# MircoWerner/VkRadixSort

Measured on AMD Instinct MI355X. Metric: Gkeys/s sorting 10^8 uint32 at 1/2/4/8 MI355X; % of HBM roofline, higher is better.
Workload: dtype u32

## Files before the change

vkradixsort_amd/csrc/vrs_contract.hip:

```cpp
#include "vrs_device.hpp"
#include "vrs_key_order.hpp"

#include <algorithm>
#include <cstdio>
#include <cstdlib>
#include <type_traits>

namespace vrs {

__device__ __forceinline__ void histogram_count(uint32_t *s_hist, uint32_t key, uint32_t shift, bool valid) {
    const uint32_t d = digit_of(key, shift);
    const uint64_t active = __ballot(valid);
    if (active == 0) return;
    const uint32_t first = static_cast<uint32_t>(__ffsll(static_cast<long long>(active))) - 1u;
    const uint32_t d0 = __builtin_amdgcn_readlane(d, first);
    const uint64_t same = __ballot(valid && d == d0);
    if (same == active) {
        if (lane_id() == first) atomicAdd(&s_hist[d0], static_cast<uint32_t>(__popcll(active)));
    } else if (valid) {
        atomicAdd(&s_hist[d], 1u);
    }
}

template <typename K, typename DG>
// ... 261 lines not shown
#pragma unroll
        for (int u = 0; u < kDepth; ++u) {
            if (r + u < q1) o[static_cast<size_t>(r + u) * kBins] = run;
            run += t[u];
        }
    }
}

constexpr uint32_t kFusedMaxChunks = 48;

template <typename K, int ITEMS, int WAVES, bool PAIRS, int RANK, int OCC, bool SPLIT = false>
__global__ __launch_bounds__(WAVES * 64, OCC) void scatter_kernel(const K *__restrict__ keys_in,
                                                             K *__restrict__ keys_out,
                                                             const uint32_t *__restrict__ values_in,
                                                             uint32_t *__restrict__ values_out,
                                                             const uint32_t *__restrict__ offsets, uint32_t n,
                                                             uint32_t shift, uint32_t W, uint32_t B, int xcd_remap,
                                                             const uint32_t *__restrict__ tile_order,
                                                             uint32_t offset_row_stride,
                                                             const K *__restrict__ splitters, uint32_t num_splitters) {
    using DG = typename std::conditional<SPLIT, SplitDigit<K>, RadixDigit<K>>::type;
    __shared__ ChunkSmem<K, ITEMS, WAVES, PAIRS> sm;
    __shared__ K s_split[SPLIT ? 256 : 1];
    DG dg;
    if constexpr (SPLIT) {
        stage_splitters(s_split, splitters, num_splitters);
        dg.splitters = s_split;
        dg.count = num_splitters;
    } else {
        dg.shift = shift;
    }
    const uint32_t w = tile_order ? tile_order[blockIdx.x]
                                  : (xcd_remap ? xcd_contiguous_tile(blockIdx.x, W) : blockIdx.x);
    const uint64_t tile_begin = static_cast<uint64_t>(w) * B * kThreads;
    if (tile_begin >= n) return;
    const uint64_t tile_keys = static_cast<uint64_t>(B) * kThreads;
    const uint32_t tile_len = static_cast<uint32_t>(tile_begin + tile_keys <= n ? tile_keys : n - tile_begin);
    uint32_t run_off =
        threadIdx.x < kBins ? offsets[static_cast<size_t>(w) * offset_row_stride * kBins + threadIdx.x] : 0u;
    constexpr uint32_t kChunk = ITEMS * WAVES * 64;
    const bool stream_in = static_cast<size_t>(n) * sizeof(K) >= kStreamInBytes;
    for (uint32_t c0 = 0; c0 < tile_len; c0 += kChunk) {
        const uint32_t valid = min(kChunk, tile_len - c0);
        const K *kin = keys_in + tile_begin + c0;
        const uint32_t *vin = PAIRS ? values_in + tile_begin + c0 : nullptr;
        if (valid == kChunk)
// ... 315 lines not shown
```

vkradixsort_amd/csrc/vrs_device.hpp:

```cpp
#pragma once
#include "vrs_kernels.h"

#include <hip/hip_ext.h>

#include <type_traits>

#define VRS_LAUNCH(kernel, grid, block, stream, ev, ...)                                                        \
    do {                                                                                                        \
        if ((ev).start != nullptr || (ev).stop != nullptr)                                                      \
            hipExtLaunchKernelGGL(kernel, grid, block, 0, stream, (ev).start, (ev).stop, 0, __VA_ARGS__);       \
        else                                                                                                    \
            hipLaunchKernelGGL(kernel, grid, block, 0, stream, __VA_ARGS__);                                    \
    } while (0)

#ifndef VRS_MARK
#define VRS_MARK(i)
#define VRS_MARK_FLUSH()
#endif
namespace vrs {

constexpr size_t kStreamInBytes = size_t(128) << 20;

constexpr int kDtUnroll = 8;
constexpr int kLbItems = 16;
constexpr int kLbBatch = 4;
constexpr int kLbWaves = 8;

constexpr int kBins = 256;
constexpr int kThreads = 256;
constexpr int kWaves = kThreads / 64;

__device__ __forceinline__ uint32_t lane_id() {
    return __builtin_amdgcn_mbcnt_hi(~0u, __builtin_amdgcn_mbcnt_lo(~0u, 0u));
}

__device__ __forceinline__ uint32_t opaque(uint32_t x) {
    asm volatile("" : "+v"(x));
    return x;
}

// ... 248 lines not shown
    mutable bool reserved_yet = false;

    __device__ __forceinline__ void publish(uint32_t v) const {
        if (reserved_yet) return;
        reserved_yet = true;
        const uint32_t cnt = v - pad_keys;
        if (cnt) {
            if (foreign) {
                const uint32_t taken = cnt + __hip_atomic_fetch_add(back, cnt, __ATOMIC_RELAXED, __HIP_MEMORY_SCOPE_AGENT);
                reserved = region_len >= taken ? region_len - taken : 0u;
            } else
                reserved = __hip_atomic_fetch_add(cursor, cnt, __ATOMIC_RELAXED, __HIP_MEMORY_SCOPE_WORKGROUP);
        }
    }
    __device__ __forceinline__ void fetch(int, uint32_t (&)[kLbBatch]) const {}
    __device__ __forceinline__ uint32_t resolve(uint32_t (&)[kLbBatch], bool &) const { return reserved; }
};

template <typename K, typename DG>
__device__ __forceinline__ void recount_keys(uint32_t *cnt, const K *keys, uint32_t count, const DG &dg) {
    for (uint32_t j = threadIdx.x; j < count; j += blockDim.x) atomicAdd(&cnt[dg(keys[j])], 1u);
}

template <typename K, int ITEMS, int WAVES, bool PAIRS, int RANK, bool FULL, typename DG, typename LB = NoLookback, typename SRC = NoPieces>
__device__ __forceinline__ void scatter_chunk(ChunkSmem<K, ITEMS, WAVES, PAIRS> &sm, const K *kin,
                                              const uint32_t *vin, K *kout, uint32_t *vout,
                                              uint32_t valid, const DG &dg, uint32_t &run_off, const LB lb = {},
                                              const SRC src = {}, bool stream_in = false) {
    constexpr uint32_t THREADS = WAVES * 64;
    const uint32_t tid = threadIdx.x;
    const uint32_t lane = tid & 63u;
    const uint32_t wave = tid >> 6;

    VRS_MARK(0);
    K key[ITEMS];
    uint32_t val[PAIRS ? ITEMS : 1];
    const uint32_t seg = wave * (ITEMS * 64) + lane;
    if (FULL && !SRC::kEnabled && stream_in) {
#pragma unroll
        for (int i = 0; i < ITEMS; ++i) key[i] = __builtin_nontemporal_load(kin + seg + i * 64);
        if constexpr (PAIRS) {
#pragma unroll
            for (int i = 0; i < ITEMS; ++i) val[i] = __builtin_nontemporal_load(vin + seg + i * 64);
        }
    } else if constexpr (SRC::kEnabled) {
        uint32_t vs[ITEMS];
#pragma unroll
        for (int i = 0; i < ITEMS; ++i) vs[i] = src.first_slot;
#pragma unroll 1
        for (uint32_t p = src.p0; p < src.p1; ++p) {
            const uint32_t lo = __builtin_amdgcn_readlane(src.lo, p), len = __builtin_amdgcn_readlane(src.len, p), vd = __builtin_amdgcn_readlane(src.slot, p);
#pragma unroll
            for (int i = 0; i < ITEMS; ++i) {
                const uint32_t idx = seg + i * 64;
                vs[i] = idx - lo < len ? vd + (idx - lo) : vs[i];
            }
        }
#pragma unroll
        for (int i = 0; i < ITEMS; ++i) {
            const K k = *src.at(vs[i]);
            key[i] = (FULL || seg + i * 64 < valid) ? k : dg.template pad<K>();
        }
        if constexpr (PAIRS) {
#pragma unroll
            for (int i = 0; i < ITEMS; ++i) val[i] = *src.val_at(vs[i]);
        }
    } else {
#pragma unroll
        for (int i = 0; i < ITEMS; ++i) {
            const uint32_t idx = seg + i * 64;
            if constexpr (FULL) {
                key[i] = kin[idx];
            } else {
                const K k = kin[idx < valid ? idx : valid - 1u];
                key[i] = idx < valid ? k : dg.template pad<K>();
            }
        }
        if constexpr (PAIRS) {
#pragma unroll
            for (int i = 0; i < ITEMS; ++i) {
                const uint32_t idx = seg + i * 64;
                val[i] = vin[FULL ? idx : (idx < valid ? idx : valid - 1u)];
            }
        }
    }
    {
        uint32_t *z = &sm.whist[0][0];
#pragma unroll
        for (int v = 0; v < 4; ++v) z[v * THREADS + tid] = 0;
        if constexpr (LB::kEnabled) {
            if (tid == 0) sm.lb_gave_up = 0;
        }
    }
    __syncthreads();
    VRS_MARK(1);

    uint32_t rank[ITEMS];
    uint32_t *my_hist = sm.whist[wave];
    if constexpr (RANK == RANK_ATOMIC) {
#pragma unroll
        for (int i = 0; i < ITEMS; ++i) {
            const uint32_t d = dg(key[i]);
            const uint32_t d0 = __builtin_amdgcn_readfirstlane(d);
            if (__ballot(d == d0) == ~0ull) {
                uint32_t old = 0;
                if (lane == 0u)
                    old = __hip_atomic_fetch_add(&my_hist[d0], 64u, __ATOMIC_RELAXED, __HIP_MEMORY_SCOPE_WORKGROUP);
                rank[i] = __builtin_amdgcn_readfirstlane(old) + lane;
// ... 111 lines not shown
        lb.template store<K, ITEMS, THREADS, FULL>(sm.gbase, key, dst, kout, valid, dg);
    } else {
#pragma unroll
        for (int i = 0; i < ITEMS; ++i) {
            if (FULL || i * THREADS + tid < valid) kout[dst[i]] = key[i];
        }
    }
    VRS_MARK(5);

    if constexpr (PAIRS) {
#pragma unroll
        for (int i = 0; i < ITEMS; ++i) val[i] = sm.vals[i * THREADS + tid];
        if constexpr (LB::kPool) {
            lb.template store_values<ITEMS, THREADS, FULL>(val, dst, vout, valid);
        } else {
#pragma unroll
            for (int i = 0; i < ITEMS; ++i) {
                if (FULL || i * THREADS + tid < valid) vout[dst[i]] = val[i];
            }
        }
    }
}

constexpr uint32_t kMsdBits = 14, kMsdBuckets = 1u << kMsdBits;
constexpr uint32_t kMsdMinShift = 13, kMsdMaxShift = 18;
constexpr uint32_t kMsdProbeWord = kMsdBuckets + 8u * 256u, kMsdOverWord = kMsdProbeWord + 1u;
constexpr uint32_t kMsdSubBits = kMsdBits - 8, kMsdSub = 1u << kMsdSubBits;

struct BitsDigit {
    uint32_t shift, mask, base;
    __device__ __forceinline__ uint32_t operator()(uint32_t key) const { return ((key - base) >> shift) & mask; }
    __device__ __forceinline__ uint32_t operator()(uint64_t key) const { return static_cast<uint32_t>(key >> shift) & mask; }
    template <typename KK>
    __device__ __forceinline__ KK pad() const { return sizeof(KK) == 4 ? static_cast<KK>(base - 1u) : static_cast<KK>(~static_cast<KK>(0)); }
};

}
```

vkradixsort_amd/csrc/vrs_msd_pool.hip:

```cpp
#include "vrs_local_sort.hpp"

#include <algorithm>
#include <cmath>

namespace vrs {

namespace {

constexpr uint32_t kPoolMinShift = 13, kPoolMaxShift = 18;
constexpr float kPoolSigmas = 6.0f;

__global__ __launch_bounds__(256) void pool_sample_kernel(const uint32_t *__restrict__ keys, uint32_t n, uint32_t key_base,
                                                          PoolStreams ps, PoolPlan *__restrict__ pool, uint32_t top_bits) {
    constexpr int kPerWave = kPoolSampleTiles / 4;
    constexpr int kLoads = kPoolSampleKeys / 64;
    __shared__ uint32_t s_hist[2][256];
    __shared__ uint32_t s_or;
    const uint32_t tid = threadIdx.x, lane = tid & 63u, wave = tid >> 6;
    s_hist[0][tid] = 0;
    s_hist[1][tid] = 0;
    if (tid == 0) s_or = 0;
    const uint32_t t0 = blockIdx.x * kPoolSampleTiles;
    const uint32_t s0 = t0 / ps.tiles_per_stream;
    uint32_t k[kPerWave][kLoads];
// ... 106 lines not shown
    static constexpr bool kPool = true;
    bool foreign = false;
    uint32_t recounted = 0;
    int index = 0;
    const void *stream_keys = nullptr;
    uint32_t done = 0;
    uint32_t seed = 0;
    uint32_t *cursor = nullptr;
    const uint32_t *region = nullptr;
    uint32_t pad_keys = 0;
    uint32_t n_virt = 0;
    uint32_t *overflow = nullptr;
    uint32_t overflow_last = 0;
    uint32_t *gbase2 = nullptr, *split = nullptr, *flags = nullptr;
    uint32_t *fail_word = nullptr;
    mutable uint32_t reserved = 0, cnt = 0, rb = 0, rc = 0, ob = 0, oc = 0;
    mutable bool reserved_yet = false;

    __device__ __forceinline__ void publish(uint32_t v) const {
        if (reserved_yet) return;
        reserved_yet = true;
        cnt = v - pad_keys;
        if (cnt) reserved = __hip_atomic_fetch_add(cursor, cnt, __ATOMIC_RELAXED, __HIP_MEMORY_SCOPE_WORKGROUP);
        rb = region[0];
        rc = region[8 * 256];
        ob = region[16 * 256];
        oc = region[24 * 256];
    }
    __device__ __forceinline__ void fetch(int, uint32_t (&)[kLbBatch]) const {}
    __device__ __forceinline__ uint32_t resolve(uint32_t (&)[kLbBatch], bool &) const { return reserved; }
    __device__ __forceinline__ void refuse() const {}
    __device__ __forceinline__ void place(uint32_t *gbase, uint32_t tid, uint32_t, uint32_t excl) const { place_run(gbase, tid, reserved, excl); }
    __device__ __forceinline__ void place_run(uint32_t *gbase, uint32_t tid, uint32_t reserved, uint32_t excl) const {
        const uint32_t end = reserved + cnt;
        uint32_t g, g2 = 0, sp = 0xFFFFFFFFu;
        bool bad = false;
        if (end <= rc) {
            g = rb + reserved - excl;
        } else if (reserved >= rc) {
            bad = end - rc > oc;
            g = n_virt + ob + (reserved - rc) - excl;
        } else {
            bad = end - rc > oc;
            sp = excl + (rc - reserved);
            g = rb + reserved - excl;
            g2 = n_virt + ob - sp;
            atomicOr(flags, 1u);
        }
        if (cnt && bad) __hip_atomic_fetch_or(fail_word, 1u, __ATOMIC_RELAXED, __HIP_MEMORY_SCOPE_AGENT);
        gbase[tid] = g;
        gbase2[tid] = g2;
        split[tid] = sp;
    }
    template <typename K, int ITEMS, uint32_t THREADS, bool FULL, typename DG>
    __device__ __forceinline__ void store(const uint32_t *, const K (&key)[ITEMS], uint32_t (&dst)[ITEMS], K *kout, uint32_t valid, const DG &dg) const {
        const uint32_t tid = threadIdx.x;
        if (*flags & 1u) {
#pragma unroll
            for (int i = 0; i < ITEMS; ++i) {
                const uint32_t d = dg(key[i]);
                if (i * THREADS + tid >= split[d]) dst[i] = gbase2[d] + (i * THREADS + tid);
            }
        }
#pragma unroll
        for (int i = 0; i < ITEMS; ++i) {
            K *p = dst[i] < n_virt ? kout + dst[i] : overflow + min(dst[i] - n_virt, overflow_last);
            if (FULL || i * THREADS + tid < valid) *p = key[i];
        }
    }
    uint32_t *overflow_values = nullptr;
    template <int ITEMS, uint32_t THREADS, bool FULL>
    __device__ __forceinline__ void store_values(const uint32_t (&val)[ITEMS], const uint32_t (&dst)[ITEMS], uint32_t *vout, uint32_t valid) const {
        const uint32_t tid = threadIdx.x;
#pragma unroll
        for (int i = 0; i < ITEMS; ++i) {
            uint32_t *p = dst[i] < n_virt ? vout + dst[i] : overflow_values + min(dst[i] - n_virt, overflow_last);
            if (FULL || i * THREADS + tid < valid) *p = val[i];
        }
    }
};

struct PoolLookback : StreamLookback {
    static constexpr bool kPool = true;
    PoolReserve at;
    __device__ __forceinline__ void publish(uint32_t v) const {
        if (!at.reserved_yet) {
            at.reserved_yet = true;
            at.cnt = v - at.pad_keys;
            if (at.cnt) __hip_atomic_fetch_add(at.cursor, at.cnt, __ATOMIC_RELAXED, __HIP_MEMORY_SCOPE_WORKGROUP);
            at.rb = at.region[0];
            at.rc = at.region[8 * 256];
            at.ob = at.region[16 * 256];
            at.oc = at.region[24 * 256];
        }
        StreamLookback::publish(v);
    }
    __device__ __forceinline__ void refuse() const { __hip_atomic_fetch_or(at.fail_word, 1u, __ATOMIC_RELAXED, __HIP_MEMORY_SCOPE_AGENT); }
    __device__ __forceinline__ void place(uint32_t *gbase, uint32_t tid, uint32_t before, uint32_t excl) const { at.place_run(gbase, tid, before, excl); }
    template <typename K, int ITEMS, uint32_t THREADS, bool FULL, typename DG>
    __device__ __forceinline__ void store(const uint32_t *g, const K (&key)[ITEMS], uint32_t (&dst)[ITEMS], K *kout, uint32_t valid, const DG &dg) const {
        at.template store<K, ITEMS, THREADS, FULL>(g, key, dst, kout, valid, dg);
    }
    template <int ITEMS, uint32_t THREADS, bool FULL>
    __device__ __forceinline__ void store_values(const uint32_t (&val)[ITEMS], const uint32_t (&dst)[ITEMS], uint32_t *vout, uint32_t valid) const {
        at.template store_values<ITEMS, THREADS, FULL>(val, dst, vout, valid);
    }
};

__device__ __forceinline__ uint32_t xcc_place(unsigned long long xcc_map) {
    const uint32_t my_xcc = xcc_id();
    uint32_t x = 8u;
#pragma unroll
    for (uint32_t q = 0; q < 8u; ++q)
        if (x == 8u && xcc_of(xcc_map, q) == my_xcc) x = q;
    return x;
}

template <bool PAIRS>
__global__ __launch_bounds__(512, 4) void pool_pass_a_kernel(const uint32_t *__restrict__ keys_in, uint32_t *__restrict__ keys_out,
                                                             uint32_t *__restrict__ overflow, uint32_t n, uint32_t key_base,
                                                             PoolStreams ps, PoolPlan *__restrict__ pool, MsdPlan *__restrict__ msd,
                                                             unsigned long long xcc_map, int misplace, uint32_t overflow_capacity, uint32_t par,
                                                             PoolPayloads pv, uint32_t top_bits) {
    __shared__ ChunkSmem<uint32_t, 16, 8, PAIRS> sm;
    __shared__ uint32_t s_gbase2[kBins], s_split[kBins], s_flags;
    if (pool->armed == 0u) return;
    const uint32_t i = blockIdx.x >> 3;
    const uint32_t s_out = xcc_place(xcc_map);
    if (s_out == 8u) {
        if (threadIdx.x == 0) __hip_atomic_fetch_or(&pool->fail[par], 1u, __ATOMIC_RELAXED, __HIP_MEMORY_SCOPE_AGENT);
        return;
    }
    if (threadIdx.x == 0) __hip_atomic_fetch_add(&pool->claim_a[s_out * kPoolMaxTilesA + i], 1u, __ATOMIC_RELAXED, __HIP_MEMORY_SCOPE_WORKGROUP);
    const uint32_t s_in = (s_out + (misplace ? (i & 1u) : 0u)) & 7u;
    const uint32_t len = ps.len[s_in];
    const uint32_t done = i * kPoolTile;
    if (done >= len) return;
    if (threadIdx.x == 0) s_flags = 0;
    const uint32_t valid = min(kPoolTile, len - done);
    const uint32_t *kin = keys_in + ps.start[s_in] + done;
    const uint32_t d = threadIdx.x & 255u;
    RadixDigit<uint32_t> dg;
    dg.shift = pool->shift + (kMsdBits - top_bits);
    dg.base = key_base;
    PoolReserve at;
    at.cursor = &msd->cursor_a[s_out][d];
    at.region = &pool->base[s_out][d];
    at.pad_keys = d == dg(dg.template pad<uint32_t>()) ? kPoolTile - valid : 0u;
    at.n_virt = n;
    at.overflow = overflow;
    at.overflow_last = overflow_capacity - 1u;
    at.gbase2 = s_gbase2;
    at.split = s_split;
    at.flags = &s_flags;
    at.fail_word = &pool->fail[par];
    uint32_t unused = 0;
    const bool stream_in = static_cast<size_t>(n) * sizeof(uint32_t) >= kStreamInBytes;
    if constexpr (PAIRS) {
        at.overflow_values = pv.overflow_values;
        PoolLookback lb;
        lb.at = at;
        lb.stream_keys = keys_in + ps.start[s_in];
        lb.done = done;
        lb.col = pv.status + static_cast<size_t>(s_out) * kBins + d;
        lb.stride = static_cast<size_t>(8) * kBins;
        lb.index = static_cast<int>(i);
        lb.tag = 1u << kLbTagShift;
        lb.budget = pv.spin_budget;
        lb.hold = pv.hold_tile >= 0 && i == static_cast<uint32_t>(pv.hold_tile);
        const uint32_t *vin = pv.values_home + ps.start[s_in] + done;
        if (valid == kPoolTile)
            scatter_chunk<uint32_t, 16, 8, true, RANK_ATOMIC, true>(sm, kin, vin, keys_out, pv.values_partner, valid, dg, unused, lb, NoPieces{}, stream_in);
        else
            scatter_chunk<uint32_t, 16, 8, true, RANK_ATOMIC, false>(sm, kin, vin, keys_out, pv.values_partner, valid, dg, unused, lb);
    } else {
        if (valid == kPoolTile)
            scatter_chunk<uint32_t, 16, 8, false, RANK_ATOMIC, true>(sm, kin, nullptr, keys_out, nullptr, valid, dg, unused, at, NoPieces{}, stream_in);
        else
            scatter_chunk<uint32_t, 16, 8, false, RANK_ATOMIC, false>(sm, kin, nullptr, keys_out, nullptr, valid, dg, unused, at);
    }
}

constexpr float kPoolR = 40.0f;
template <uint32_t SUB>
__device__ __forceinline__ uint32_t pool_space(uint32_t c) {
    if (c == 0u) return 0u;
    const float x = static_cast<float>(c), s = static_cast<float>(SUB);
    return (c + static_cast<uint32_t>(kPoolSigmas * sqrtf(s * kPoolR * (x + s * kPoolR))) + SUB * (kPoolRoomFloor + 4u) + 3u) & ~3u;
}
template <uint32_t SUBBITS, bool GROUPED>
__global__ __launch_bounds__(512) void pool_plan_kernel(MsdPlan *__restrict__ msd, PoolPlan *__restrict__ pool, uint32_t n, uint32_t tiles_b_cap,
                                                       uint32_t slack_capacity, const uint32_t *__restrict__ regions, const uint32_t *__restrict__ overflow,
                                                       uint32_t key_base, PoolStreams ps, PoolGroups groups, uint32_t par, uint32_t keep, uint32_t top_bits) {
    constexpr uint32_t THREADS = 512, WAVES = THREADS / 64, SUB = 1u << SUBBITS, PER = SUB / 64u;
    __shared__ uint32_t s_c[kBins];
    __shared__ uint32_t s_red[4][WAVES];
    __shared__ uint32_t s_hist[WAVES][SUB];
    __shared__ uint2 s_piece[16];
    __shared__ uint32_t s_first[17];
    __shared__ uint32_t s_bad;
    const uint32_t tid = threadIdx.x, lane = tid & 63u, wave = tid >> 6, a = blockIdx.x;
    const uint32_t shift = GROUPED ? 18u : pool->shift, bshift = shift + kMsdBits - top_bits - SUBBITS;
    if (!GROUPED && tid < 256u) {
// ... 194 lines not shown
                                 ? 1u
                                 : 0u;
            pool->max_bucket = 0;
            pool->fail[par ^ 1u] = 0;
            if constexpr (GROUPED) pool->shift = shift;
            msd->shift = shift;
            msd->sub_bits = SUBBITS;
            msd->ok = 0;
        }
    }
}

struct SlackReserve {
    static constexpr bool kEnabled = true;
    static constexpr bool kReserves = true;
    static constexpr bool kPool = true;
    bool foreign = false;
    uint32_t recounted = 0;
    int index = 0;
    const void *stream_keys = nullptr;
    uint32_t done = 0;
    uint32_t seed = 0;
    uint32_t *cursor = nullptr;
    uint32_t start = 0, cap = 0;
    uint32_t local_cap = 0;
    uint32_t *max_bucket = nullptr;
    uint32_t dump = 0;
    uint32_t pad_keys = 0;
    uint32_t above = 0, key_base = 0;
    uint32_t *fail_word = nullptr;
    mutable uint32_t reserved = 0, cnt = 0;
    mutable bool reserved_yet = false;

    __device__ __forceinline__ void publish(uint32_t v) const {
        if (reserved_yet) return;
        reserved_yet = true;
        cnt = v - pad_keys;
        if (cnt) reserved = __hip_atomic_fetch_add(cursor, cnt, __ATOMIC_RELAXED, __HIP_MEMORY_SCOPE_WORKGROUP);
    }
    __device__ __forceinline__ void fetch(int, uint32_t (&)[kLbBatch]) const {}
    __device__ __forceinline__ uint32_t resolve(uint32_t (&)[kLbBatch], bool &) const { return reserved; }
    __device__ __forceinline__ void refuse() const {}
    __device__ __forceinline__ void place(uint32_t *gbase, uint32_t tid, uint32_t, uint32_t excl) const { place_run(gbase, tid, reserved, excl); }
    __device__ __forceinline__ void place_run(uint32_t *gbase, uint32_t tid, uint32_t reserved, uint32_t excl) const {
        const uint32_t end = reserved + cnt;
        const bool bad = cnt != 0u && end > cap;
        if (bad) {
            __hip_atomic_fetch_or(fail_word, 1u, __ATOMIC_RELAXED, __HIP_MEMORY_SCOPE_AGENT);
        } else if (cnt != 0u && end > local_cap) {
            __hip_atomic_fetch_or(fail_word, 2u, __ATOMIC_RELAXED, __HIP_MEMORY_SCOPE_AGENT);
            __hip_atomic_fetch_max(max_bucket, end, __ATOMIC_RELAXED, __HIP_MEMORY_SCOPE_AGENT);
        }
        gbase[tid] = (bad ? dump : start + reserved) - excl;
    }
    template <typename K, int ITEMS, uint32_t THREADS, bool FULL, typename DG>
    __device__ __forceinline__ void store(const uint32_t *, const K (&key)[ITEMS], uint32_t (&dst)[ITEMS], K *kout, uint32_t valid, const DG &) const {
        const uint32_t tid = threadIdx.x;
        uint32_t over = 0;
#pragma unroll
        for (int i = 0; i < ITEMS; ++i) {
            if (FULL || i * THREADS + tid < valid) {
                over |= (key[i] - key_base) & above;
                kout[dst[i]] = key[i];
            }
        }
        if (__ballot(over != 0u) != 0ull && (tid & 63u) == 0u) __hip_atomic_fetch_or(fail_word, 1u, __ATOMIC_RELAXED, __HIP_MEMORY_SCOPE_AGENT);
    }
    template <int ITEMS, uint32_t THREADS, bool FULL>
    __device__ __forceinline__ void store_values(const uint32_t (&val)[ITEMS], const uint32_t (&dst)[ITEMS], uint32_t *vout, uint32_t valid) const {
// ... 14 lines not shown
            if (at.cnt) __hip_atomic_fetch_add(at.cursor, at.cnt, __ATOMIC_RELAXED, __HIP_MEMORY_SCOPE_WORKGROUP);
        }
        StreamLookback::publish(v);
    }
    __device__ __forceinline__ void refuse() const { __hip_atomic_fetch_or(at.fail_word, 1u, __ATOMIC_RELAXED, __HIP_MEMORY_SCOPE_AGENT); }
    __device__ __forceinline__ void place(uint32_t *gbase, uint32_t tid, uint32_t before, uint32_t excl) const { at.place_run(gbase, tid, before, excl); }
    template <typename K, int ITEMS, uint32_t THREADS, bool FULL, typename DG>
    __device__ __forceinline__ void store(const uint32_t *g, const K (&key)[ITEMS], uint32_t (&dst)[ITEMS], K *kout, uint32_t valid, const DG &dg) const {
        at.template store<K, ITEMS, THREADS, FULL>(g, key, dst, kout, valid, dg);
    }
    template <int ITEMS, uint32_t THREADS, bool FULL>
    __device__ __forceinline__ void store_values(const uint32_t (&val)[ITEMS], const uint32_t (&dst)[ITEMS], uint32_t *vout, uint32_t valid) const {
        at.template store_values<ITEMS, THREADS, FULL>(val, dst, vout, valid);
    }
};

template <uint32_t SUBBITS, bool PAIRS>
__global__ __launch_bounds__(512, PAIRS ? 4 : 6) void pool_pass_b_kernel(const uint32_t *__restrict__ regions, const uint32_t *__restrict__ overflow,
                                                             uint32_t *__restrict__ slack, const MsdPlan *__restrict__ msd, PoolPlan *__restrict__ pool,
                                                             uint32_t n_virt, uint32_t key_base, uint32_t local_cap, uint32_t dump,
                                                             unsigned long long xcc_map, uint32_t stamp, uint32_t grouped, uint32_t par, PoolPayloads pv,
                                                             uint32_t top_bits) {
    __shared__ ChunkSmem<uint32_t, 16, 8, PAIRS> sm;
    const uint32_t x = xcc_place(xcc_map), j = blockIdx.x >> 3;
    if (pool->ok_a == 0u) return;
    if (x == 8u) {
        if (threadIdx.x == 0) __hip_atomic_fetch_or(&pool->fail[par], 1u, __ATOMIC_RELAXED, __HIP_MEMORY_SCOPE_AGENT);
        return;
    }
    uint32_t claimed = 0;
    if (threadIdx.x == 0) claimed = __hip_atomic_exchange(&pool->claim_b[j * 8u + x], stamp, __ATOMIC_RELAXED, __HIP_MEMORY_SCOPE_WORKGROUP);
    const uint2 entry = pool->tile_map[x][j < kPoolMaxTilesB ? j : 0u];
    if (j >= pool->tiles_b[x][32]) return;
    const uint32_t a = entry.y & 255u, tile_lo = (entry.y >> 8) * kPoolTile;
    const bool one_piece = entry.x != kPoolTileGeneral;
    const uint32_t lane = threadIdx.x & 63u;
    uint2 pc = make_uint2(0, 0);
    if (!one_piece) pc = pool->pieces[a][lane & 15u];
    const uint32_t shift = pool->shift;
    constexpr uint32_t SUB = 1u << SUBBITS;
    const uint32_t d = threadIdx.x & 255u, b = a * SUB + min(d, SUB - 1u);
    SlackReserve at;
    at.cursor = &pool->sub_cursor[b];
    if (threadIdx.x < SUB) {
        at.start = pool->sub_start[b];
        at.cap = pool->sub_start[b + 1u] - at.start;
    }
    at.local_cap = local_cap;
    at.max_bucket = &pool->max_bucket;
    const uint32_t pend = pc.x, pslot = pc.y;
    const uint32_t before = __shfl_up(pend, 1);
    const uint32_t plo = lane == 0u ? 0u : before;
    const uint32_t plen = lane < 16u ? pend - plo : 0u;
    const uint32_t keys_a = __builtin_amdgcn_readlane(pend, 15);
    const uint32_t valid = one_piece ? kPoolTile : min(kPoolTile, keys_a - tile_lo);
    const unsigned long long touch = __ballot(plen != 0u && plo < tile_lo + valid && pend > tile_lo);
    PieceSrc src;
    src.p0 = static_cast<uint32_t>(__builtin_ctzll(touch | (1ull << 63)));
    src.p1 = 64u - static_cast<uint32_t>(__builtin_clzll(touch | 1ull));
    src.lo = plo - tile_lo;
    src.len = plen;
    src.slot = pslot;
    src.regions = regions;
    src.overflow = overflow;
    src.n_virt = n_virt;
    const uint32_t slot0 = one_piece ? entry.x : __builtin_amdgcn_readlane(pslot, src.p0) + (tile_lo - __builtin_amdgcn_readlane(plo, src.p0));
    src.first_slot = slot0;
    const BitsDigit dg{shift + kMsdBits - top_bits - SUBBITS, SUB - 1u, key_base};
    at.dump = dump;
    at.pad_keys = d == SUB - 1u ? kPoolTile - valid : 0u;
    at.above = grouped ? 0xFF000000u : (shift + kMsdBits < 32u ? ~0u << (shift + kMsdBits) : 0u);
    at.key_base = grouped ? key_base + (a << 24) : key_base;
    at.fail_word = &pool->fail[par];
    uint32_t unused = 0;
    if (threadIdx.x == 0 && claimed == stamp) __hip_atomic_fetch_or(&pool->fail[par], 1u, __ATOMIC_RELAXED, __HIP_MEMORY_SCOPE_AGENT);
    const bool stream_in = static_cast<size_t>(pool->top_base[256]) * sizeof(uint32_t) >= kStreamInBytes;
    const uint32_t *kin = slot0 < n_virt ? regions + slot0 : overflow + (slot0 - n_virt);
    if constexpr (PAIRS) {
        src.vregions = pv.values_partner;
        src.voverflow = pv.overflow_values;
        SlackLookback lb;
        lb.at = at;
        lb.col = pv.status + (static_cast<size_t>(j - (entry.y >> 8)) * 8u + x) * kBins + d;
        lb.stride = static_cast<size_t>(8) * kBins;
        lb.index = static_cast<int>(entry.y >> 8);
        lb.tag = 6u << kLbTagShift;
        lb.budget = pv.spin_budget;
        const uint32_t *vin = slot0 < n_virt ? pv.values_partner + slot0 : pv.overflow_values + (slot0 - n_virt);
        if (one_piece)
            scatter_chunk<uint32_t, 16, 8, true, RANK_ATOMIC, true, BitsDigit, SlackLookback>(sm, kin, vin, slack, pv.slack_values, valid, dg, unused, lb, NoPieces{}, stream_in);
        else if (valid == kPoolTile)
            scatter_chunk<uint32_t, 16, 8, true, RANK_ATOMIC, true, BitsDigit, SlackLookback, PieceSrc>(sm, nullptr, nullptr, slack, pv.slack_values, valid, dg, unused, lb, src);
        else
            scatter_chunk<uint32_t, 16, 8, true, RANK_ATOMIC, false, BitsDigit, SlackLookback, PieceSrc>(sm, nullptr, nullptr, slack, pv.slack_values, valid, dg, unused, lb, src);
    } else {
        if (one_piece)
            scatter_chunk<uint32_t, 16, 8, false, RANK_ATOMIC, true, BitsDigit, SlackReserve>(sm, kin, nullptr, slack, nullptr, valid, dg, unused, at, NoPieces{}, stream_in);
        else if (valid == kPoolTile)
            scatter_chunk<uint32_t, 16, 8, false, RANK_ATOMIC, true, BitsDigit, SlackReserve, PieceSrc>(sm, nullptr, nullptr, slack, nullptr, valid, dg, unused, at, src);
        else
            scatter_chunk<uint32_t, 16, 8, false, RANK_ATOMIC, false, BitsDigit, SlackReserve, PieceSrc>(sm, nullptr, nullptr, slack, nullptr, valid, dg, unused, at, src);
    }
}

}


hipError_t launch_pool_sample(hipStream_t stream, const PoolSampleArgs &a, LaunchEvents ev) {
    const uint32_t *keys = a.keys;
    const uint32_t n = a.form.n, key_base = a.form.key_base, overflow_capacity = a.overflow_capacity, par = a.form.par, top_bits = a.form.top_bits;
    const PoolStreams &ps = a.form.ps;
    PoolPlan *pool = a.form.pool;
    if (n == 0 || ps.tiles_per_stream < kPoolSampleTiles) return hipErrorInvalidValue;
    const uint32_t grid = (ps.tiles_total + kPoolSampleTiles - 1u) / kPoolSampleTiles;
    VRS_LAUNCH(pool_sample_kernel, dim3(grid), dim3(256), stream, ev, keys, n, key_base, ps, pool, top_bits);
    hipLaunchKernelGGL(pool_layout_kernel, dim3(1), dim3(256), 0, stream, ps, pool, overflow_capacity, par);
    return hipGetLastError();
}

hipError_t launch_pool_pass_a(hipStream_t stream, const PoolPassAArgs &a, LaunchEvents ev) {
    const uint32_t *keys_in = a.keys_in;
    uint32_t *keys_out = a.keys_out, *overflow = a.overflow;
    const uint32_t n = a.form.n, key_base = a.form.key_base, overflow_capacity = a.overflow_capacity, par = a.form.par, top_bits = a.form.top_bits;
    const PoolStreams &ps = a.form.ps;
    PoolPlan *pool = a.form.pool;
// ... 79 lines not shown
```

Measured before the change: 197.5.

## Issue tile key loads before plan setup in pool scatter passes

Splits scatter_chunk into a separate load step and a scatter-from-registers step. In the pool pass A and pass B kernels, the tile's keys and values are now loaded before the plan words, reservation regions and early-exit checks are read, so global load latency overlaps with the setup work. It also reads plan fields through constant-address-space scalar loads, and adds a flags==0 fast path so stores whose destination lies wholly inside the region skip the overflow/split handling. The cost is loads issued even for tiles that then exit early, extra register pressure from holding keys across the setup, and more complex control flow.

Result: faster. 200.6, median of 6 (+1.6%).

```diff
diff --git a/vkradixsort_amd/csrc/vrs_contract.hip b/vkradixsort_amd/csrc/vrs_contract.hip
--- a/vkradixsort_amd/csrc/vrs_contract.hip
+++ b/vkradixsort_amd/csrc/vrs_contract.hip
@@ -307,6 +307,7 @@
     using DG = typename std::conditional<SPLIT, SplitDigit<K>, RadixDigit<K>>::type;
     __shared__ ChunkSmem<K, ITEMS, WAVES, PAIRS> sm;
     __shared__ K s_split[SPLIT ? 256 : 1];
+    VRS_MARK(6);
     DG dg;
     if constexpr (SPLIT) {
         stage_splitters(s_split, splitters, num_splitters);
diff --git a/vkradixsort_amd/csrc/vrs_device.hpp b/vkradixsort_amd/csrc/vrs_device.hpp
--- a/vkradixsort_amd/csrc/vrs_device.hpp
+++ b/vkradixsort_amd/csrc/vrs_device.hpp
@@ -15,7 +15,7 @@
 
 #ifndef VRS_MARK
 #define VRS_MARK(i)
-#define VRS_MARK_FLUSH()
+#define VRS_MARK_FLUSH(...)
 #endif
 namespace vrs {
 
@@ -310,68 +310,46 @@
     for (uint32_t j = threadIdx.x; j < count; j += blockDim.x) atomicAdd(&cnt[dg(keys[j])], 1u);
 }
 
-template <typename K, int ITEMS, int WAVES, bool PAIRS, int RANK, bool FULL, typename DG, typename LB = NoLookback, typename SRC = NoPieces>
-__device__ __forceinline__ void scatter_chunk(ChunkSmem<K, ITEMS, WAVES, PAIRS> &sm, const K *kin,
-                                              const uint32_t *vin, K *kout, uint32_t *vout,
-                                              uint32_t valid, const DG &dg, uint32_t &run_off, const LB lb = {},
-                                              const SRC src = {}, bool stream_in = false) {
+template <typename K, int ITEMS, bool PAIRS, bool FULL>
+__device__ __forceinline__ void chunk_load(const K *kin, const uint32_t *vin, uint32_t valid, bool stream_in, K (&key)[ITEMS], uint32_t (&val)[PAIRS ? ITEMS : 1]) {
+    const uint32_t seg = (threadIdx.x >> 6) * (ITEMS * 64) + (threadIdx.x & 63u);
+    if (FULL && stream_in) {
+#pragma unroll
+        for (int i = 0; i < ITEMS; ++i) key[i] = __builtin_nontemporal_load(kin + seg + i * 64);
+        if constexpr (PAIRS) {
+#pragma unroll
+            for (int i = 0; i < ITEMS; ++i) val[i] = __builtin_nontemporal_load(vin + seg + i * 64);
+        }
+    } else {
+#pragma unroll
+        for (int i = 0; i < ITEMS; ++i) {
+            const uint32_t idx = seg + i * 64;
+            key[i] = kin[FULL ? idx : (idx < valid ? idx : valid - 1u)];
+        }
+        if constexpr (PAIRS) {
+#pragma unroll
+            for (int i = 0; i < ITEMS; ++i) {
+                const uint32_t idx = seg + i * 64;
+                val[i] = vin[FULL ? idx : (idx < valid ? idx : valid - 1u)];
+            }
+        }
+    }
+}
+template <typename K, int ITEMS, typename DG>
+__device__ __forceinline__ void chunk_pad(K (&key)[ITEMS], uint32_t valid, const DG &dg) {
+    const uint32_t seg = (threadIdx.x >> 6) * (ITEMS * 64) + (threadIdx.x & 63u);
+#pragma unroll
+    for (int i = 0; i < ITEMS; ++i) key[i] = seg + i * 64 < valid ? key[i] : dg.template pad<K>();
+}
+
+template <typename K, int ITEMS, int WAVES, bool PAIRS, int RANK, bool FULL, typename DG, typename LB = NoLookback>
+__device__ __forceinline__ void scatter_chunk_loaded(ChunkSmem<K, ITEMS, WAVES, PAIRS> &sm, K (&key)[ITEMS], uint32_t (&val)[PAIRS ? ITEMS : 1], K *kout,
+                                                     uint32_t *vout, uint32_t valid, const DG &dg, uint32_t &run_off, const LB lb = {}) {
     constexpr uint32_t THREADS = WAVES * 64;
     const uint32_t tid = threadIdx.x;
     const uint32_t lane = tid & 63u;
     const uint32_t wave = tid >> 6;
 
-    VRS_MARK(0);
-    K key[ITEMS];
-    uint32_t val[PAIRS ? ITEMS : 1];
-    const uint32_t seg = wave * (ITEMS * 64) + lane;
-    if (FULL && !SRC::kEnabled && stream_in) {
-#pragma unroll
-        for (int i = 0; i < ITEMS; ++i) key[i] = __builtin_nontemporal_load(kin + seg + i * 64);
-        if constexpr (PAIRS) {
-#pragma unroll
-            for (int i = 0; i < ITEMS; ++i) val[i] = __builtin_nontemporal_load(vin + seg + i * 64);
-        }
-    } else if constexpr (SRC::kEnabled) {
-        uint32_t vs[ITEMS];
-#pragma unroll
-        for (int i = 0; i < ITEMS; ++i) vs[i] = src.first_slot;
-#pragma unroll 1
-        for (uint32_t p = src.p0; p < src.p1; ++p) {
-            const uint32_t lo = __builtin_amdgcn_readlane(src.lo, p), len = __builtin_amdgcn_readlane(src.len, p), vd = __builtin_amdgcn_readlane(src.slot, p);
-#pragma unroll
-            for (int i = 0; i < ITEMS; ++i) {
-                const uint32_t idx = seg + i * 64;
-                vs[i] = idx - lo < len ? vd + (idx - lo) : vs[i];
-            }
-        }
-#pragma unroll
-        for (int i = 0; i < ITEMS; ++i) {
-            const K k = *src.at(vs[i]);
-            key[i] = (FULL || seg + i * 64 < valid) ? k : dg.template pad<K>();
-        }
-        if constexpr (PAIRS) {
-#pragma unroll
-            for (int i = 0; i < ITEMS; ++i) val[i] = *src.val_at(vs[i]);
-        }
-    } else {
-#pragma unroll
-        for (int i = 0; i < ITEMS; ++i) {
-            const uint32_t idx = seg + i * 64;
-            if constexpr (FULL) {
-                key[i] = kin[idx];
-            } else {
-                const K k = kin[idx < valid ? idx : valid - 1u];
-                key[i] = idx < valid ? k : dg.template pad<K>();
-            }
-        }
-        if constexpr (PAIRS) {
-#pragma unroll
-            for (int i = 0; i < ITEMS; ++i) {
-                const uint32_t idx = seg + i * 64;
-                val[i] = vin[FULL ? idx : (idx < valid ? idx : valid - 1u)];
-            }
-        }
-    }
     {
         uint32_t *z = &sm.whist[0][0];
 #pragma unroll
@@ -529,6 +507,44 @@
     }
 }
 
+template <typename K, int ITEMS, int WAVES, bool PAIRS, int RANK, bool FULL, typename DG, typename LB = NoLookback, typename SRC = NoPieces>
+__device__ __forceinline__ void scatter_chunk(ChunkSmem<K, ITEMS, WAVES, PAIRS> &sm, const K *kin,
+                                              const uint32_t *vin, K *kout, uint32_t *vout,
+                                              uint32_t valid, const DG &dg, uint32_t &run_off, const LB lb = {},
+                                              const SRC src = {}, bool stream_in = false) {
+    VRS_MARK(0);
+    K key[ITEMS];
+    uint32_t val[PAIRS ? ITEMS : 1];
+    if constexpr (SRC::kEnabled) {
+        const uint32_t seg = (threadIdx.x >> 6) * (ITEMS * 64) + (threadIdx.x & 63u);
+        uint32_t vs[ITEMS];
+#pragma unroll
+        for (int i = 0; i < ITEMS; ++i) vs[i] = src.first_slot;
+#pragma unroll 1
+        for (uint32_t p = src.p0; p < src.p1; ++p) {
+            const uint32_t lo = __builtin_amdgcn_readlane(src.lo, p), len = __builtin_amdgcn_readlane(src.len, p), vd = __builtin_amdgcn_readlane(src.slot, p);
+#pragma unroll
+            for (int i = 0; i < ITEMS; ++i) {
+                const uint32_t idx = seg + i * 64;
+                vs[i] = idx - lo < len ? vd + (idx - lo) : vs[i];
+            }
+        }
+#pragma unroll
+        for (int i = 0; i < ITEMS; ++i) {
+            const K k = *src.at(vs[i]);
+            key[i] = (FULL || seg + i * 64 < valid) ? k : dg.template pad<K>();
+        }
+        if constexpr (PAIRS) {
+#pragma unroll
+            for (int i = 0; i < ITEMS; ++i) val[i] = *src.val_at(vs[i]);
+        }
+    } else {
+        chunk_load<K, ITEMS, PAIRS, FULL>(kin, vin, valid, stream_in, key, val);
+        if constexpr (!FULL) chunk_pad(key, valid, dg);
+    }
+    scatter_chunk_loaded<K, ITEMS, WAVES, PAIRS, RANK, FULL, DG, LB>(sm, key, val, kout, vout, valid, dg, run_off, lb);
+}
+
 constexpr uint32_t kMsdBits = 14, kMsdBuckets = 1u << kMsdBits;
 constexpr uint32_t kMsdMinShift = 13, kMsdMaxShift = 18;
 constexpr uint32_t kMsdProbeWord = kMsdBuckets + 8u * 256u, kMsdOverWord = kMsdProbeWord + 1u;
diff --git a/vkradixsort_amd/csrc/vrs_msd_pool.hip b/vkradixsort_amd/csrc/vrs_msd_pool.hip
--- a/vkradixsort_amd/csrc/vrs_msd_pool.hip
+++ b/vkradixsort_amd/csrc/vrs_msd_pool.hip
@@ -152,6 +152,8 @@
         reserved_yet = true;
         cnt = v - pad_keys;
         if (cnt) reserved = __hip_atomic_fetch_add(cursor, cnt, __ATOMIC_RELAXED, __HIP_MEMORY_SCOPE_WORKGROUP);
+    }
+    __device__ __forceinline__ void load_region() {
         rb = region[0];
         rc = region[8 * 256];
         ob = region[16 * 256];
@@ -170,12 +172,13 @@
         } else if (reserved >= rc) {
             bad = end - rc > oc;
             g = n_virt + ob + (reserved - rc) - excl;
+            if (cnt) atomicOr(flags, 2u);
         } else {
             bad = end - rc > oc;
             sp = excl + (rc - reserved);
             g = rb + reserved - excl;
             g2 = n_virt + ob - sp;
-            atomicOr(flags, 1u);
+            atomicOr(flags, 3u);
         }
         if (cnt && bad) __hip_atomic_fetch_or(fail_word, 1u, __ATOMIC_RELAXED, __HIP_MEMORY_SCOPE_AGENT);
         gbase[tid] = g;
@@ -185,7 +188,14 @@
     template <typename K, int ITEMS, uint32_t THREADS, bool FULL, typename DG>
     __device__ __forceinline__ void store(const uint32_t *, const K (&key)[ITEMS], uint32_t (&dst)[ITEMS], K *kout, uint32_t valid, const DG &dg) const {
         const uint32_t tid = threadIdx.x;
-        if (*flags & 1u) {
+        const uint32_t f = *flags;
+        if (f == 0u) {
+#pragma unroll
+            for (int i = 0; i < ITEMS; ++i)
+                if (FULL || i * THREADS + tid < valid) kout[dst[i]] = key[i];
+            return;
+        }
+        if (f & 1u) {
 #pragma unroll
             for (int i = 0; i < ITEMS; ++i) {
                 const uint32_t d = dg(key[i]);
@@ -202,6 +212,12 @@
     template <int ITEMS, uint32_t THREADS, bool FULL>
     __device__ __forceinline__ void store_values(const uint32_t (&val)[ITEMS], const uint32_t (&dst)[ITEMS], uint32_t *vout, uint32_t valid) const {
         const uint32_t tid = threadIdx.x;
+        if (*flags == 0u) {
+#pragma unroll
+            for (int i = 0; i < ITEMS; ++i)
+                if (FULL || i * THREADS + tid < valid) vout[dst[i]] = val[i];
+            return;
+        }
 #pragma unroll
         for (int i = 0; i < ITEMS; ++i) {
             uint32_t *p = dst[i] < n_virt ? vout + dst[i] : overflow_values + min(dst[i] - n_virt, overflow_last);
@@ -218,10 +234,6 @@
             at.reserved_yet = true;
             at.cnt = v - at.pad_keys;
             if (at.cnt) __hip_atomic_fetch_add(at.cursor, at.cnt, __ATOMIC_RELAXED, __HIP_MEMORY_SCOPE_WORKGROUP);
-            at.rb = at.region[0];
-            at.rc = at.region[8 * 256];
-            at.ob = at.region[16 * 256];
-            at.oc = at.region[24 * 256];
         }
         StreamLookback::publish(v);
     }
@@ -244,6 +256,68 @@
     for (uint32_t q = 0; q < 8u; ++q)
         if (x == 8u && xcc_of(xcc_map, q) == my_xcc) x = q;
     return x;
+}
+
+__device__ __forceinline__ uint32_t plan_word(const uint32_t *p) {
+    return *(const uint32_t __attribute__((address_space(4))) *)(p);
+}
+__device__ __forceinline__ uint2 plan_word(const uint2 *p) {
+    typedef uint32_t pair_t __attribute__((ext_vector_type(2)));
+    const pair_t v = *(const pair_t __attribute__((address_space(4))) *)(p);
+    return make_uint2(v.x, v.y);
+}
+
+template <bool PAIRS, bool FULL>
+__device__ __forceinline__ void pool_pass_a_tile(ChunkSmem<uint32_t, 16, 8, PAIRS> &sm, uint32_t *gbase2, uint32_t *split, uint32_t *flags, const uint32_t *kin,
+                                                 const uint32_t *vin, const uint32_t *slice_keys, uint32_t *keys_out, uint32_t *overflow, uint32_t n,
+                                                 uint32_t key_base, PoolPlan *pool, MsdPlan *msd, uint32_t s_out, uint32_t i, uint32_t done, uint32_t valid,
+                                                 uint32_t armed, uint32_t shift, uint32_t overflow_capacity, uint32_t par, const PoolPayloads &pv, uint32_t top_bits) {
+    const bool stream_in = static_cast<size_t>(n) * sizeof(uint32_t) >= kStreamInBytes;
+    VRS_MARK(0);
+    uint32_t key[16], val[PAIRS ? 16 : 1];
+    chunk_load<uint32_t, 16, PAIRS, FULL>(kin, vin, valid, stream_in, key, val);
+    const uint32_t d = threadIdx.x & 255u, row = s_out & 7u;
+    PoolReserve at;
+    at.region = &pool->base[row][d];
+    at.load_region();
+    asm volatile("" : : "s"(kin), "s"(vin), "s"(pool) : "memory");
+    if (armed == 0u) return;
+    if (s_out == 8u) {
+        if (threadIdx.x == 0) __hip_atomic_fetch_or(&pool->fail[par], 1u, __ATOMIC_RELAXED, __HIP_MEMORY_SCOPE_AGENT);
+        return;
+    }
+    if (threadIdx.x == 0) __hip_atomic_fetch_add(&pool->claim_a[s_out * kPoolMaxTilesA + i], 1u, __ATOMIC_RELAXED, __HIP_MEMORY_SCOPE_WORKGROUP);
+    if (threadIdx.x == 0) *flags = 0;
+    RadixDigit<uint32_t> dg;
+    dg.shift = shift + (kMsdBits - top_bits);
+    dg.base = key_base;
+    if constexpr (!FULL) chunk_pad(key, valid, dg);
+    at.cursor = &msd->cursor_a[s_out][d];
+    at.pad_keys = d == dg(dg.template pad<uint32_t>()) ? kPoolTile - valid : 0u;
+    at.n_virt = n;
+    at.overflow = overflow;
+    at.overflow_last = overflow_capacity - 1u;
+    at.gbase2 = gbase2;
+    at.split = split;
+    at.flags = flags;
+    at.fail_word = &pool->fail[par];
+    uint32_t unused = 0;
+    if constexpr (PAIRS) {
+        at.overflow_values = pv.overflow_values;
+        PoolLookback lb;
+        lb.at = at;
+        lb.stream_keys = slice_keys;
+        lb.done = done;
+        lb.col = pv.status + static_cast<size_t>(s_out) * kBins + d;
+        lb.stride = static_cast<size_t>(8) * kBins;
+        lb.index = static_cast<int>(i);
+        lb.tag = 1u << kLbTagShift;
+        lb.budget = pv.spin_budget;
+        lb.hold = pv.hold_tile >= 0 && i == static_cast<uint32_t>(pv.hold_tile);
+        scatter_chunk_loaded<uint32_t, 16, 8, true, RANK_ATOMIC, FULL>(sm, key, val, keys_out, pv.values_partner, valid, dg, unused, lb);
+    } else {
+        scatter_chunk_loaded<uint32_t, 16, 8, false, RANK_ATOMIC, FULL>(sm, key, val, keys_out, nullptr, valid, dg, unused, at);
+    }
 }
 
 template <bool PAIRS>
@@ -254,61 +328,29 @@
                                                              PoolPayloads pv, uint32_t top_bits) {
     __shared__ ChunkSmem<uint32_t, 16, 8, PAIRS> sm;
     __shared__ uint32_t s_gbase2[kBins], s_split[kBins], s_flags;
-    if (pool->armed == 0u) return;
+    VRS_MARK(6);
+    const uint32_t armed = plan_word(&pool->armed), shift = plan_word(&pool->shift);
     const uint32_t i = blockIdx.x >> 3;
     const uint32_t s_out = xcc_place(xcc_map);
-    if (s_out == 8u) {
-        if (threadIdx.x == 0) __hip_atomic_fetch_or(&pool->fail[par], 1u, __ATOMIC_RELAXED, __HIP_MEMORY_SCOPE_AGENT);
-        return;
-    }
-    if (threadIdx.x == 0) __hip_atomic_fetch_add(&pool->claim_a[s_out * kPoolMaxTilesA + i], 1u, __ATOMIC_RELAXED, __HIP_MEMORY_SCOPE_WORKGROUP);
     const uint32_t s_in = (s_out + (misplace ? (i & 1u) : 0u)) & 7u;
     const uint32_t len = ps.len[s_in];
     const uint32_t done = i * kPoolTile;
-    if (done >= len) return;
-    if (threadIdx.x == 0) s_flags = 0;
-    const uint32_t valid = min(kPoolTile, len - done);
-    const uint32_t *kin = keys_in + ps.start[s_in] + done;
-    const uint32_t d = threadIdx.x & 255u;
-    RadixDigit<uint32_t> dg;
-    dg.shift = pool->shift + (kMsdBits - top_bits);
-    dg.base = key_base;
-    PoolReserve at;
-    at.cursor = &msd->cursor_a[s_out][d];
-    at.region = &pool->base[s_out][d];
-    at.pad_keys = d == dg(dg.template pad<uint32_t>()) ? kPoolTile - valid : 0u;
-    at.n_virt = n;
-    at.overflow = overflow;
-    at.overflow_last = overflow_capacity - 1u;
-    at.gbase2 = s_gbase2;
-    at.split = s_split;
-    at.flags = &s_flags;
-    at.fail_word = &pool->fail[par];
-    uint32_t unused = 0;
-    const bool stream_in = static_cast<size_t>(n) * sizeof(uint32_t) >= kStreamInBytes;
-    if constexpr (PAIRS) {
-        at.overflow_values = pv.overflow_values;
-        PoolLookback lb;
-        lb.at = at;
-        lb.stream_keys = keys_in + ps.start[s_in];
-        lb.done = done;
-        lb.col = pv.status + static_cast<size_t>(s_out) * kBins + d;
-        lb.stride = static_cast<size_t>(8) * kBins;
-        lb.index = static_cast<int>(i);
-        lb.tag = 1u << kLbTagShift;
-        lb.budget = pv.spin_budget;
-        lb.hold = pv.hold_tile >= 0 && i == static_cast<uint32_t>(pv.hold_tile);
-        const uint32_t *vin = pv.values_home + ps.start[s_in] + done;
-        if (valid == kPoolTile)
-            scatter_chunk<uint32_t, 16, 8, true, RANK_ATOMIC, true>(sm, kin, vin, keys_out, pv.values_partner, valid, dg, unused, lb, NoPieces{}, stream_in);
-        else
-            scatter_chunk<uint32_t, 16, 8, true, RANK_ATOMIC, false>(sm, kin, vin, keys_out, pv.values_partner, valid, dg, unused, lb);
-    } else {
-        if (valid == kPoolTile)
-            scatter_chunk<uint32_t, 16, 8, false, RANK_ATOMIC, true>(sm, kin, nullptr, keys_out, nullptr, valid, dg, unused, at, NoPieces{}, stream_in);
-        else
-            scatter_chunk<uint32_t, 16, 8, false, RANK_ATOMIC, false>(sm, kin, nullptr, keys_out, nullptr, valid, dg, unused, at);
-    }
+    const uint32_t valid = done < len ? min(kPoolTile, len - done) : 0u;
+    const uint32_t *slice_keys = keys_in + ps.start[s_in];
+    const uint32_t *vin = PAIRS ? pv.values_home + ps.start[s_in] + done : nullptr;
+    if (valid == kPoolTile)
+        pool_pass_a_tile<PAIRS, true>(sm, s_gbase2, s_split, &s_flags, slice_keys + done, vin, slice_keys, keys_out, overflow, n, key_base, pool, msd, s_out, i,
+                                      done, valid, armed, shift, overflow_capacity, par, pv, top_bits);
+    else if (valid != 0u)
+        pool_pass_a_tile<PAIRS, false>(sm, s_gbase2, s_split, &s_flags, slice_keys + done, vin, slice_keys, keys_out, overflow, n, key_base, pool, msd, s_out, i,
+                                       done, valid, armed, shift, overflow_capacity, par, pv, top_bits);
+    else if (armed != 0u) {
+        if (s_out == 8u) {
+            if (threadIdx.x == 0) __hip_atomic_fetch_or(&pool->fail[par], 1u, __ATOMIC_RELAXED, __HIP_MEMORY_SCOPE_AGENT);
+        } else if (threadIdx.x == 0)
+            __hip_atomic_fetch_add(&pool->claim_a[s_out * kPoolMaxTilesA + i], 1u, __ATOMIC_RELAXED, __HIP_MEMORY_SCOPE_WORKGROUP);
+    }
+    VRS_MARK_FLUSH(1);
 }
 
 constexpr float kPoolR = 40.0f;
@@ -549,7 +591,7 @@
     uint32_t done = 0;
     uint32_t seed = 0;
     uint32_t *cursor = nullptr;
-    uint32_t start = 0, cap = 0;
+    uint32_t start = 0, next = 0;
     uint32_t local_cap = 0;
     uint32_t *max_bucket = nullptr;
     uint32_t dump = 0;
@@ -571,7 +613,7 @@
     __device__ __forceinline__ void place(uint32_t *gbase, uint32_t tid, uint32_t, uint32_t excl) const { place_run(gbase, tid, reserved, excl); }
     __device__ __forceinline__ void place_run(uint32_t *gbase, uint32_t tid, uint32_t reserved, uint32_t excl) const {
         const uint32_t end = reserved + cnt;
-        const bool bad = cnt != 0u && end > cap;
+        const bool bad = cnt != 0u && end > next - start;
         if (bad) {
             __hip_atomic_fetch_or(fail_word, 1u, __ATOMIC_RELAXED, __HIP_MEMORY_SCOPE_AGENT);
         } else if (cnt != 0u && end > local_cap) {
@@ -632,38 +674,78 @@
                                                              unsigned long long xcc_map, uint32_t stamp, uint32_t grouped, uint32_t par, PoolPayloads pv,
                                                              uint32_t top_bits) {
     __shared__ ChunkSmem<uint32_t, 16, 8, PAIRS> sm;
-    const uint32_t x = xcc_place(xcc_map), j = blockIdx.x >> 3;
-    if (pool->ok_a == 0u) return;
+    VRS_MARK(6);
+    const uint32_t x = xcc_place(xcc_map), xs = x & 7u, j = blockIdx.x >> 3;
+    const uint32_t ok_a = plan_word(&pool->ok_a), tiles = plan_word(&pool->tiles_b[xs][32]);
+    const uint2 entry = plan_word(&pool->tile_map[xs][j < kPoolMaxTilesB ? j : 0u]);
+    const uint32_t total = plan_word(&pool->top_base[256]), shift = plan_word(&pool->shift);
+    asm volatile("" : : "s"(ok_a), "s"(tiles), "s"(entry.x), "s"(entry.y), "s"(total), "s"(shift), "s"(regions), "s"(overflow), "s"(slack), "s"(n_virt), "s"(stamp),
+                 "s"(top_bits), "s"(key_base), "s"(local_cap), "s"(dump), "s"(grouped), "s"(par)
+                 : "memory");
+    if (ok_a == 0u) return;
     if (x == 8u) {
         if (threadIdx.x == 0) __hip_atomic_fetch_or(&pool->fail[par], 1u, __ATOMIC_RELAXED, __HIP_MEMORY_SCOPE_AGENT);
         return;
     }
     uint32_t claimed = 0;
     if (threadIdx.x == 0) claimed = __hip_atomic_exchange(&pool->claim_b[j * 8u + x], stamp, __ATOMIC_RELAXED, __HIP_MEMORY_SCOPE_WORKGROUP);
-    const uint2 entry = pool->tile_map[x][j < kPoolMaxTilesB ? j : 0u];
-    if (j >= pool->tiles_b[x][32]) return;
+    if (j >= tiles) return;
     const uint32_t a = entry.y & 255u, tile_lo = (entry.y >> 8) * kPoolTile;
     const bool one_piece = entry.x != kPoolTileGeneral;
-    const uint32_t lane = threadIdx.x & 63u;
-    uint2 pc = make_uint2(0, 0);
-    if (!one_piece) pc = pool->pieces[a][lane & 15u];
-    const uint32_t shift = pool->shift;
+    const bool stream_in = static_cast<size_t>(total) * sizeof(uint32_t) >= kStreamInBytes;
     constexpr uint32_t SUB = 1u << SUBBITS;
     const uint32_t d = threadIdx.x & 255u, b = a * SUB + min(d, SUB - 1u);
+    const BitsDigit dg{shift + kMsdBits - top_bits - SUBBITS, SUB - 1u, key_base};
     SlackReserve at;
-    at.cursor = &pool->sub_cursor[b];
-    if (threadIdx.x < SUB) {
+    auto set_up = [&](uint32_t valid) {
+        at.cursor = &pool->sub_cursor[b];
         at.start = pool->sub_start[b];
-        at.cap = pool->sub_start[b + 1u] - at.start;
-    }
-    at.local_cap = local_cap;
-    at.max_bucket = &pool->max_bucket;
+        at.next = pool->sub_start[b + 1u];
+        at.local_cap = local_cap;
+        at.max_bucket = &pool->max_bucket;
+        at.dump = dump;
+        at.pad_keys = d == SUB - 1u ? kPoolTile - valid : 0u;
+        at.above = grouped ? 0xFF000000u : (shift + kMsdBits < 32u ? ~0u << (shift + kMsdBits) : 0u);
+        at.key_base = grouped ? key_base + (a << 24) : key_base;
+        at.fail_word = &pool->fail[par];
+        if (threadIdx.x == 0 && claimed == stamp) __hip_atomic_fetch_or(&pool->fail[par], 1u, __ATOMIC_RELAXED, __HIP_MEMORY_SCOPE_AGENT);
+    };
+    auto chain = [&](SlackLookback &lb) {
+        lb.at = at;
+        lb.col = pv.status + (static_cast<size_t>(j - (entry.y >> 8)) * 8u + x) * kBins + d;
+        lb.stride = static_cast<size_t>(8) * kBins;
+        lb.index = static_cast<int>(entry.y >> 8);
+        lb.tag = 6u << kLbTagShift;
+        lb.budget = pv.spin_budget;
+    };
+    uint32_t unused = 0;
+    if (one_piece) {
+        const uint32_t slot0 = entry.x;
+        const uint32_t *kin = slot0 < n_virt ? regions + slot0 : overflow + (slot0 - n_virt);
+        const uint32_t *vin = !PAIRS ? nullptr : slot0 < n_virt ? pv.values_partner + slot0 : pv.overflow_values + (slot0 - n_virt);
+        VRS_MARK(0);
+        uint32_t key[16], val[PAIRS ? 16 : 1];
+        chunk_load<uint32_t, 16, PAIRS, true>(kin, vin, kPoolTile, stream_in, key, val);
+        asm volatile("" : "+v"(claimed) : : "memory");
+        set_up(kPoolTile);
+        if constexpr (PAIRS) {
+            SlackLookback lb;
+            chain(lb);
+            scatter_chunk_loaded<uint32_t, 16, 8, true, RANK_ATOMIC, true, BitsDigit, SlackLookback>(sm, key, val, slack, pv.slack_values, kPoolTile, dg, unused, lb);
+        } else {
+            scatter_chunk_loaded<uint32_t, 16, 8, false, RANK_ATOMIC, true, BitsDigit, SlackReserve>(sm, key, val, slack, nullptr, kPoolTile, dg, unused, at);
+        }
+        VRS_MARK_FLUSH(2);
+        return;
+    }
+    const uint32_t lane = threadIdx.x & 63u;
+    const uint2 pc = pool->pieces[a][lane & 15u];
     const uint32_t pend = pc.x, pslot = pc.y;
     const uint32_t before = __shfl_up(pend, 1);
     const uint32_t plo = lane == 0u ? 0u : before;
     const uint32_t plen = lane < 16u ? pend - plo : 0u;
     const uint32_t keys_a = __builtin_amdgcn_readlane(pend, 15);
-    const uint32_t valid = one_piece ? kPoolTile : min(kPoolTile, keys_a - tile_lo);
+    const uint32_t valid = min(kPoolTile, keys_a - tile_lo);
     const unsigned long long touch = __ballot(plen != 0u && plo < tile_lo + valid && pend > tile_lo);
     PieceSrc src;
     src.p0 = static_cast<uint32_t>(__builtin_ctzll(touch | (1ull << 63)));
@@ -674,43 +756,24 @@
     src.regions = regions;
     src.overflow = overflow;
     src.n_virt = n_virt;
-    const uint32_t slot0 = one_piece ? entry.x : __builtin_amdgcn_readlane(pslot, src.p0) + (tile_lo - __builtin_amdgcn_readlane(plo, src.p0));
-    src.first_slot = slot0;
-    const BitsDigit dg{shift + kMsdBits - top_bits - SUBBITS, SUB - 1u, key_base};
-    at.dump = dump;
-    at.pad_keys = d == SUB - 1u ? kPoolTile - valid : 0u;
-    at.above = grouped ? 0xFF000000u : (shift + kMsdBits < 32u ? ~0u << (shift + kMsdBits) : 0u);
-    at.key_base = grouped ? key_base + (a << 24) : key_base;
-    at.fail_word = &pool->fail[par];
-    uint32_t unused = 0;
-    if (threadIdx.x == 0 && claimed == stamp) __hip_atomic_fetch_or(&pool->fail[par], 1u, __ATOMIC_RELAXED, __HIP_MEMORY_SCOPE_AGENT);
-    const bool stream_in = static_cast<size_t>(pool->top_base[256]) * sizeof(uint32_t) >= kStreamInBytes;
-    const uint32_t *kin = slot0 < n_virt ? regions + slot0 : overflow + (slot0 - n_virt);
+    src.first_slot = __builtin_amdgcn_readlane(pslot, src.p0) + (tile_lo - __builtin_amdgcn_readlane(plo, src.p0));
+    set_up(valid);
     if constexpr (PAIRS) {
         src.vregions = pv.values_partner;
         src.voverflow = pv.overflow_values;
         SlackLookback lb;
-        lb.at = at;
-        lb.col = pv.status + (static_cast<size_t>(j - (entry.y >> 8)) * 8u + x) * kBins + d;
-        lb.stride = static_cast<size_t>(8) * kBins;
-        lb.index = static_cast<int>(entry.y >> 8);
-        lb.tag = 6u << kLbTagShift;
-        lb.budget = pv.spin_budget;
-        const uint32_t *vin = slot0 < n_virt ? pv.values_partner + slot0 : pv.overflow_values + (slot0 - n_virt);
-        if (one_piece)
-            scatter_chunk<uint32_t, 16, 8, true, RANK_ATOMIC, true, BitsDigit, SlackLookback>(sm, kin, vin, slack, pv.slack_values, valid, dg, unused, lb, NoPieces{}, stream_in);
-        else if (valid == kPoolTile)
+        chain(lb);
+        if (valid == kPoolTile)
             scatter_chunk<uint32_t, 16, 8, true, RANK_ATOMIC, true, BitsDigit, SlackLookback, PieceSrc>(sm, nullptr, nullptr, slack, pv.slack_values, valid, dg, unused, lb, src);
         else
             scatter_chunk<uint32_t, 16, 8, true, RANK_ATOMIC, false, BitsDigit, SlackLookback, PieceSrc>(sm, nullptr, nullptr, slack, pv.slack_values, valid, dg, unused, lb, src);
     } else {
-        if (one_piece)
-            scatter_chunk<uint32_t, 16, 8, false, RANK_ATOMIC, true, BitsDigit, SlackReserve>(sm, kin, nullptr, slack, nullptr, valid, dg, unused, at, NoPieces{}, stream_in);
-        else if (valid == kPoolTile)
+        if (valid == kPoolTile)
             scatter_chunk<uint32_t, 16, 8, false, RANK_ATOMIC, true, BitsDigit, SlackReserve, PieceSrc>(sm, nullptr, nullptr, slack, nullptr, valid, dg, unused, at, src);
         else
             scatter_chunk<uint32_t, 16, 8, false, RANK_ATOMIC, false, BitsDigit, SlackReserve, PieceSrc>(sm, nullptr, nullptr, slack, nullptr, valid, dg, unused, at, src);
     }
+    VRS_MARK_FLUSH(2);
 }
 
 }
```
